# dbolya/yolact

Measured on AMD Instinct MI355X. Metric: images/sec (550x550, batch 8 per GPU), YOLACT yolact_resnet50 forward + Detect (Fast NMS), higher is better.
Workload: dtype f32 (fp32 in / fp32 accumulate / fp32 out; 93 % of the GEMM time on fp16x2 tiles = every fp32 operand as two fp16 pieces by round to nearest (22 significant bits + 2 signs: exact for ~2/3 of all fp32 values, one fp32 ulp otherwise), 3 exact piece products per product on the fp16 matrix pipe; measure

## Files before the change

yolact_amd/csrc/wgemm.hip:

```cpp
#include "common.h"
#include <stdlib.h>
#include <type_traits>
#include "../../include/yolact_amd.h"

int ymi_internal_prof_begin(double flops, int tile, int kind, hipStream_t s);
void ymi_internal_prof_end(int idx, hipStream_t s);

namespace {

typedef __attribute__((address_space(3))) void *lds_ptr_t;
typedef _Float16 f16x8 __attribute__((ext_vector_type(8)));
typedef unsigned u32x4 __attribute__((ext_vector_type(4)));
constexpr unsigned OOB = 0x80000000u;

constexpr int BM = 128, BN = 256;
constexpr int A_BYTES = 2 * BM * 64, B_BYTES = 2 * BN * 64, STAGE = A_BYTES + B_BYTES, NST = 3;
constexpr int OFF_SC = NST * STAGE, WG_LDS = OFF_SC + 2 * BN * 4;
constexpr int NPC = 12;

struct WgParams {
  const char *v, *u;
  const float *uinv, *x_amax;
  float *m;
  long v_gs, u_gs, m_gs;
  unsigned v_plane, u_plane;
  int G, T, C, Ng, cout_pad, tiles_m, tiles_n, nitems;
  float amax_mul;
  unsigned long long *trace;
  int abl;
};

__global__ __launch_bounds__(512, 2) void wgemm_k(const WgParams p) {
#if defined(__HIP_DEVICE_COMPILE__)
  __shared__ __attribute__((aligned(16))) char lds[WG_LDS];
  const int t = threadIdx.x, lane = t & 63, wave = __builtin_amdgcn_readfirstlane(t >> 6);
  const bool producer = wave >= 4;
  const int lr = lane & 31, hh = lane >> 5;
  const int nk = p.C >> 5;
  const int nb = (int)gridDim.x, b0 = (int)blockIdx.x;
  const int my_items = (p.nitems - b0 + nb - 1) / nb;
  const int nsteps = my_items * nk;
#ifdef YMI_DIAGNOSTICS
  unsigned long long tr_[8] = {0, 0, 0, 0, 0, 0, 0, 0};
  const bool tracing = p.trace != nullptr;
  tr_[0] = __builtin_amdgcn_s_memtime();
#endif
#define WG_WAIT_VM(N) asm volatile("s_waitcnt vmcnt(%0)" ::"n"(N) : "memory")
#define WG_BARRIER() asm volatile("s_waitcnt lgkmcnt(0)\n\ts_barrier" ::: "memory")
  auto decode = [&](int it, int &g, int &tm, int &tn) {
    tn = it % p.tiles_n;
    const int r = it / p.tiles_n;
    tm = r % p.tiles_m;
    g = r / p.tiles_m;
  };

  if (producer) {
    const int pw = wave - 4;
    int a_row[4], a_dst[4], b_row[8], b_dst[8];
    unsigned a_ko[4], b_ko[8];
#pragma unroll
    for (int i = 0; i < 4; ++i) {
      const int q = pw + 4 * i, plane = q >> 3, rg = q & 7;
      const int row = rg * 16 + (lane >> 2), lsl = (lane & 3) ^ ((row >> 2) & 3);
      a_row[i] = row; a_ko[i] = (unsigned)plane * p.v_plane + 16u * lsl; a_dst[i] = plane * (BM * 64) + rg * 1024;
    }
#pragma unroll
    for (int i = 0; i < 8; ++i) {
      const int q = pw + 4 * i, plane = q >> 4, rg = q & 15;
      const int row = rg * 16 + (lane >> 2), lsl = (lane & 3) ^ ((row >> 2) & 3);
      b_row[i] = row; b_ko[i] = (unsigned)plane * p.u_plane + 16u * lsl; b_dst[i] = A_BYTES + plane * (BN * 64) + rg * 1024;
    }
    int ridx = 0, rkc = 0;
    __amdgpu_buffer_rsrc_t vrs, urs, srs;
    unsigned a_vo[4], b_vo[8];
    int sc_par = 0;
    auto open_item = [&](int idx) {
      const bool live = idx < my_items;
      int g = 0, tm = 0, tn = 0;
      decode(live ? b0 + idx * nb : 0, g, tm, tn);
      vrs = __builtin_amdgcn_make_buffer_rsrc((void *)(p.v + (size_t)g * p.v_gs), 0, live ? (int)p.v_gs : 0, 0x00020000);
      urs = __builtin_amdgcn_make_buffer_rsrc((void *)(p.u + (size_t)g * p.u_gs), 0, live ? (int)p.u_gs : 0, 0x00020000);
      srs = __builtin_amdgcn_make_buffer_rsrc((void *)(p.uinv + (size_t)g * p.cout_pad), 0, live ? p.cout_pad * 4 : 0, 0x00020000);
#pragma unroll
      for (int i = 0; i < 4; ++i) {
        const int row = tm * BM + a_row[i];
        a_vo[i] = (live && row < p.T && !(p.abl & 2)) ? a_ko[i] + (unsigned)(row * p.C) * 2u : OOB;
      }
#pragma unroll
      for (int i = 0; i < 8; ++i) {
        const int row = tn * BN + b_row[i];
        b_vo[i] = (live && row < p.cout_pad && !(p.abl & 4)) ? b_ko[i] + (unsigned)(row * p.C) * 2u : OOB;
      }
      const int n = tn * BN + 4 * lane;
      __builtin_amdgcn_raw_ptr_buffer_load_lds(srs, (lds_ptr_t)(lds + OFF_SC + sc_par * (BN * 4)), 16, (live && n < p.cout_pad) ? (unsigned)n * 4u : OOB, 0, 0, 0);
      sc_par ^= 1;
    };
    auto request = [&](int stage) {
      if (rkc == 0) open_item(ridx);
      char *dst = lds + stage * STAGE;
      const unsigned so = (unsigned)rkc * 64u;
#pragma unroll
      for (int i = 0; i < 4; ++i) __builtin_amdgcn_raw_ptr_buffer_load_lds(vrs, (lds_ptr_t)(dst + a_dst[i]), 16, a_vo[i], so, 0, 0);
#pragma unroll
      for (int i = 0; i < 8; ++i) __builtin_amdgcn_raw_ptr_buffer_load_lds(urs, (lds_ptr_t)(dst + b_dst[i]), 16, b_vo[i], so, 0, 0);
      if (++rkc == nk) { rkc = 0; ++ridx; }
    };
    request(0);
    request(1);
    WG_WAIT_VM(NPC);
#ifdef YMI_DIAGNOSTICS
    tr_[1] = __builtin_amdgcn_s_memtime();
#endif
    WG_BARRIER();
    int st = 2;
    for (int s = 0; s < nsteps; ++s) {
      request(st);
      st = st == 2 ? 0 : st + 1;
#ifdef YMI_DIAGNOSTICS
      const unsigned long long a_ = tracing ? __builtin_amdgcn_s_memtime() : 0ull;
#endif
      WG_WAIT_VM(NPC);
#ifdef YMI_DIAGNOSTICS
      const unsigned long long b_ = tracing ? __builtin_amdgcn_s_memtime() : 0ull;
#endif
      WG_BARRIER();
#ifdef YMI_DIAGNOSTICS
      if (tracing) { tr_[2] += b_ - a_; tr_[3] += __builtin_amdgcn_s_memtime() - b_; }
#endif
    }
    WG_WAIT_VM(0);
  } else {
    const int wc = wave & 1, wp = wave >> 1;
    const int psw = (lr >> 2) & 3;
    float sA, invA;
    ymi_h2_scale(ymi_amax_read(p.x_amax) * p.amax_mul, sA, invA);
    f32x16 acc[4][2];
#pragma unroll
    for (int i = 0; i < 4; ++i)
#pragma unroll
      for (int j = 0; j < 2; ++j)
#pragma unroll
        for (int r = 0; r < 16; ++r) acc[i][j][r] = 0.f;
    const int uo0 = A_BYTES + (32 * (4 * wc) + lr) * 64 + 16 * ((0 + hh) ^ psw), uo1 = A_BYTES + (32 * (4 * wc) + lr) * 64 + 16 * ((2 + hh) ^ psw);
    const int vo0 = (32 * (2 * wp) + lr) * 64 + 16 * ((0 + hh) ^ psw), vo1 = (32 * (2 * wp) + lr) * 64 + 16 * ((2 + hh) ^ psw);
#ifdef YMI_DIAGNOSTICS
    tr_[1] = __builtin_amdgcn_s_memtime();
#endif
    WG_BARRIER();
    __builtin_amdgcn_s_setprio(1);
    int st = 0, kc = 0, idx = 0, sc_par = 0;
    for (int s = 0; s < nsteps; ++s) {
      const char *sb = lds + st * STAGE;
#pragma unroll
      for (int s2 = 0; s2 < 2; ++s2) {
        const char *ub = sb + (s2 ? uo1 : uo0), *vb = sb + (s2 ? vo1 : vo0);
        f16x8 vh[2], vl[2];
#pragma unroll
        for (int j = 0; j < 2; ++j) {
          vh[j] = *reinterpret_cast<const f16x8 *>(vb + j * 2048);
          vl[j] = *reinterpret_cast<const f16x8 *>(vb + BM * 64 + j * 2048);
        }
#pragma unroll
        for (int ip = 0; ip < 2; ++ip) {
          f16x8 uh[2], ul[2];
#pragma unroll
          for (int ii = 0; ii < 2; ++ii) {
            uh[ii] = *reinterpret_cast<const f16x8 *>(ub + (2 * ip + ii) * 2048);
            ul[ii] = *reinterpret_cast<const f16x8 *>(ub + BN * 64 + (2 * ip + ii) * 2048);
          }
#pragma unroll
          for (int pr = 0; pr < 3; ++pr)
#pragma unroll
            for (int ii = 0; ii < 2; ++ii)
#pragma unroll
              for (int j = 0; j < 2; ++j)
#ifdef YMI_DIAGNOSTICS
                if (!(p.abl & 8))
#endif
                acc[2 * ip + ii][j] = __builtin_amdgcn_mfma_f32_32x32x16_f16(pr == 0 ? ul[ii] : uh[ii], pr == 1 ? vl[j] : vh[j], acc[2 * ip + ii][j], 0, 0, 0);
        }
      }
      st = st == 2 ? 0 : st + 1;
      if (++kc == nk) {
        kc = 0;
        int g, tm, tn;
        decode(b0 + idx * nb, g, tm, tn);
        ++idx;
        const float *sc = reinterpret_cast<const float *>(lds + OFF_SC + sc_par * (BN * 4));
        sc_par ^= 1;
        float *mg = p.m + (size_t)g * p.m_gs;
#pragma unroll
        for (int j = 0; j < 2; ++j) {
          const int row = tm * BM + 32 * (2 * wp + j) + lr;
          const bool rok = row < p.T;
#pragma unroll
          for (int i = 0; i < 4; ++i)
#pragma unroll
            for (int gq = 0; gq < 4; ++gq) {
              const int nl = 32 * (4 * wc + i) + 8 * gq + 4 * hh, n = tn * BN + nl;
              const f32x4 s4 = *reinterpret_cast<const f32x4 *>(sc + nl);
              f32x4 v;
#pragma unroll
              for (int e = 0; e < 4; ++e) { v[e] = acc[i][j][4 * gq + e] * (s4[e] * invA); acc[i][j][4 * gq + e] = 0.f; }
#ifdef YMI_DIAGNOSTICS
              if (p.abl & 1) continue;
              if (p.abl & 16) { if (rok && n < p.Ng) __builtin_nontemporal_store(v, reinterpret_cast<f32x4 *>(mg + (size_t)row * p.Ng + n)); continue; }
#endif
              if (rok && n < p.Ng) *reinterpret_cast<f32x4 *>(mg + (size_t)row * p.Ng + n) = v;
            }
        }
      }
#ifdef YMI_DIAGNOSTICS
      const unsigned long long a_ = tracing ? __builtin_amdgcn_s_memtime() : 0ull;
#endif
      WG_BARRIER();
#ifdef YMI_DIAGNOSTICS
      if (tracing) tr_[3] += __builtin_amdgcn_s_memtime() - a_;
#endif
    }
    __builtin_amdgcn_s_setprio(0);
  }
#undef WG_WAIT_VM
#undef WG_BARRIER
#ifdef YMI_DIAGNOSTICS
  if (tracing) {
    asm volatile("s_waitcnt vmcnt(0)" ::: "memory");
    tr_[5] = __builtin_amdgcn_s_memtime();
    if (lane == 0 && (wave == 0 || wave == 4)) {
      unsigned long long *o_ = p.trace + 32 * (size_t)blockIdx.x + (wave == 0 ? 0 : 16);
#pragma unroll
      for (int i = 0; i < 8; ++i) o_[i] = tr_[i];
      o_[14] = (unsigned long long)nsteps;
      o_[15] = 1;
    }
  }
#endif
#endif
}

}

int ymi_internal_wgemm(const void *v, const void *u, const float *uinv, const float *x_amax, float amax_mul, float *m, int G, long T,
                       int C, int Ng, int cout_pad, double prof_flops, int prof_kind, hipStream_t s) {
  if (!v || !u || !uinv || !x_amax || !m) return YMI_ENULL;
  if (C % 32 != 0 || C < 64 || (Ng & 3) || G <= 0 || T <= 0) return YMI_ESHAPE;
  if (T * (long)C * 4 >= (1L << 31) || (long)cout_pad * C * 4 >= (1L << 31) || T * (long)Ng >= (1L << 29)) return YMI_ESHAPE;
  if ((((uintptr_t)v) | ((uintptr_t)u) | ((uintptr_t)m) | ((uintptr_t)uinv)) & 15) return YMI_ESHAPE;
  WgParams p;
  p.v = (const char *)v; p.u = (const char *)u; p.uinv = uinv; p.x_amax = x_amax; p.m = m;
  p.v_plane = (unsigned)(T * C * 2); p.v_gs = 2L * T * C * 2;
  p.u_plane = (unsigned)((long)cout_pad * C * 2); p.u_gs = 2L * cout_pad * C * 2;
  p.m_gs = T * (long)Ng;
  p.G = G; p.T = (int)T; p.C = C; p.Ng = Ng; p.cout_pad = cout_pad;
  p.tiles_m = (int)((T + BM - 1) / BM); p.tiles_n = (Ng + BN - 1) / BN; p.nitems = G * p.tiles_m * p.tiles_n;
  p.amax_mul = amax_mul;
  p.trace = nullptr; p.abl = 0;
#ifdef YMI_DIAGNOSTICS
  { const char *e = getenv("YMI_WGEMM_ABLATE"); p.abl = e ? atoi(e) : 0; }
  { const char *e = getenv("YMI_WGEMM_TRACE"); p.trace = e ? (unsigned long long *)strtoull(e, nullptr, 0) : nullptr; }
#endif
  int dev = 0, cus = 256;
  hipGetDevice(&dev);
  hipDeviceGetAttribute(&cus, hipDeviceAttributeMultiprocessorCount, dev);
  const int pr = ymi_internal_prof_begin(prof_flops, YMI_TILE_H2 | YMI_TILE_WG_128x256, prof_kind, s);
  hipLaunchKernelGGL(wgemm_k, dim3((unsigned)(p.nitems < cus ? p.nitems : cus)), dim3(512), 0, s, p);
  const int rc = ymi_launch_status();
  ymi_internal_prof_end(pr, s);
  return rc;
}
```

Before: 2307.

## Add weight-stationary wgemm variant keeping U tile in registers for small C

Adds a second GEMM kernel for C of 64, 128 or 256. Each block holds its 256-column slice of the weight operand (U) in registers for the whole K range and streams a contiguous range of M tiles, so weights are loaded once per block instead of once per output tile. The host picks this path when its per-block tile count is not much worse than the round-robin scheduler's, and an environment variable can force the old path. The cost is heavy register use for the resident U fragments (lower occupancy, 256 threads with no producer waves) and possible load imbalance when M tiles split unevenly across blocks.

After: 2349 (median of 6 runs). +1.8%, better.

```diff
diff --git a/yolact_amd/csrc/wgemm.hip b/yolact_amd/csrc/wgemm.hip
--- a/yolact_amd/csrc/wgemm.hip
+++ b/yolact_amd/csrc/wgemm.hip
@@ -1,4 +1,5 @@
 #include "common.h"
+#include <stdio.h>
 #include <stdlib.h>
 #include <type_traits>
 #include "../../include/yolact_amd.h"
@@ -25,6 +26,7 @@
   long v_gs, u_gs, m_gs;
   unsigned v_plane, u_plane;
   int G, T, C, Ng, cout_pad, tiles_m, tiles_n, nitems;
+  int bpc;
   float amax_mul;
   unsigned long long *trace;
   int abl;
@@ -232,6 +234,205 @@
       for (int i = 0; i < 8; ++i) o_[i] = tr_[i];
       o_[14] = (unsigned long long)nsteps;
       o_[15] = 1;
+    }
+  }
+#endif
+#endif
+}
+
+constexpr int US_NST = 3, US_OFF_SC = US_NST * A_BYTES, US_OFF_U = US_OFF_SC + BN * 4, US_LDS = US_OFF_U + US_NST * B_BYTES;
+constexpr int US_NPC = 4;
+
+template <int NK, bool NOMFMA = false>
+__global__ __launch_bounds__(256) void wgemm_us_k(const WgParams p) {
+#if defined(__HIP_DEVICE_COMPILE__)
+  __shared__ __attribute__((aligned(16))) char lds[US_LDS];
+  const int t = threadIdx.x, lane = t & 63, wave = __builtin_amdgcn_readfirstlane(t >> 6);
+  const int lr = lane & 31, hh = lane >> 5;
+  const int lb = ymi_xcd_remap((int)blockIdx.x, (int)gridDim.x);
+  const int gc = lb / p.bpc, jb = lb % p.bpc;
+  const int g = gc / p.tiles_n, tn = gc % p.tiles_n;
+  const int tm0 = jb * p.tiles_m / p.bpc, tm1 = (jb + 1) * p.tiles_m / p.bpc;
+#ifdef YMI_DIAGNOSTICS
+  unsigned long long tr_[8] = {0, 0, 0, 0, 0, 0, 0, 0};
+  const bool tracing = p.trace != nullptr;
+  tr_[0] = __builtin_amdgcn_s_memtime();
+#endif
+#define WG_WAIT_VM(N) asm volatile("s_waitcnt vmcnt(%0)" ::"n"(N) : "memory")
+#define WG_BARRIER() asm volatile("s_waitcnt lgkmcnt(0)\n\ts_barrier" ::: "memory")
+  int a_row[4], a_dst[4];
+  unsigned a_ko[4], a_vo[4], a_vn[4];
+#pragma unroll
+  for (int i = 0; i < 4; ++i) {
+    const int q = wave + 4 * i, plane = q >> 3, rg = q & 7;
+    const int row = rg * 16 + (lane >> 2), lsl = (lane & 3) ^ ((row >> 2) & 3);
+    a_row[i] = row; a_ko[i] = (unsigned)plane * p.v_plane + 16u * lsl; a_dst[i] = plane * (BM * 64) + rg * 1024;
+  }
+  const __amdgpu_buffer_rsrc_t vrs = __builtin_amdgcn_make_buffer_rsrc((void *)(p.v + (size_t)g * p.v_gs), 0, (int)p.v_gs, 0x00020000);
+  auto tile_offsets = [&](int tm, unsigned (&vo)[4]) {
+#pragma unroll
+    for (int i = 0; i < 4; ++i) {
+      const int row = tm * BM + a_row[i];
+      vo[i] = (tm < tm1 && row < p.T && !(p.abl & 2)) ? a_ko[i] + (unsigned)(row * p.C) * 2u : OOB;
+    }
+  };
+  auto piece = [&](int stage, const unsigned (&vo)[4], int kc, int i) {
+    __builtin_amdgcn_raw_ptr_buffer_load_lds(vrs, (lds_ptr_t)(lds + stage * A_BYTES + a_dst[i]), 16, vo[i], (unsigned)kc * 64u, 0, 0);
+  };
+  auto request = [&](int stage, const unsigned (&vo)[4], int kc) {
+#pragma unroll
+    for (int i = 0; i < 4; ++i) piece(stage, vo, kc, i);
+  };
+  if (t < 64) {
+    const int n = tn * BN + 4 * t;
+    f32x4 s4 = {0.f, 0.f, 0.f, 0.f};
+    if (n < p.cout_pad) s4 = *reinterpret_cast<const f32x4 *>(p.uinv + (size_t)g * p.cout_pad + n);
+    *reinterpret_cast<f32x4 *>(lds + US_OFF_SC + 16 * t) = s4;
+  }
+  f16x8 u[2][2][2 * NK];
+  const __amdgpu_buffer_rsrc_t urs = __builtin_amdgcn_make_buffer_rsrc((void *)(p.u + (size_t)g * p.u_gs), 0, (int)p.u_gs, 0x00020000);
+  int b_dst[8];
+  unsigned b_vo[8];
+#pragma unroll
+  for (int i = 0; i < 8; ++i) {
+    const int q = wave + 4 * i, plane = q >> 4, rg = q & 15;
+    const int row = rg * 16 + (lane >> 2), lsl = (lane & 3) ^ ((row >> 2) & 3), grow = tn * BN + row;
+    b_dst[i] = plane * (BN * 64) + rg * 1024;
+    b_vo[i] = (grow < p.cout_pad && !(p.abl & 4)) ? (unsigned)plane * p.u_plane + 16u * lsl + (unsigned)(grow * p.C) * 2u : OOB;
+  }
+  auto upiece = [&](int stage, int kc, int i) {
+    __builtin_amdgcn_raw_ptr_buffer_load_lds(urs, (lds_ptr_t)(lds + US_OFF_U + stage * B_BYTES + b_dst[i]), 16, b_vo[i], (unsigned)kc * 64u, 0, 0);
+  };
+  tile_offsets(tm0, a_vo);
+#pragma unroll
+  for (int c = 0; c < 2; ++c) {
+    request(c, a_vo, c);
+#pragma unroll
+    for (int i = 0; i < 8; ++i) upiece(c, c, i);
+  }
+  float sA, invA;
+  ymi_h2_scale(ymi_amax_read(p.x_amax) * p.amax_mul, sA, invA);
+  f32x16 acc[2][4];
+#pragma unroll
+  for (int i = 0; i < 2; ++i)
+#pragma unroll
+    for (int j = 0; j < 4; ++j)
+#pragma unroll
+      for (int r = 0; r < 16; ++r) acc[i][j][r] = 0.f;
+  const int psw = (lr >> 2) & 3;
+  const int vo0 = lr * 64 + 16 * ((0 + hh) ^ psw), vo1 = lr * 64 + 16 * ((2 + hh) ^ psw);
+  const float *sc = reinterpret_cast<const float *>(lds + US_OFF_SC);
+  float *mg = p.m + (size_t)g * p.m_gs;
+  WG_WAIT_VM(0);
+#ifdef YMI_DIAGNOSTICS
+  tr_[1] = __builtin_amdgcn_s_memtime();
+#endif
+  WG_BARRIER();
+  __builtin_amdgcn_s_setprio(1);
+  f16x8 fa[4], fb[4];
+  auto rd = [&](f16x8 (&f)[4], int stage, int s2, int jp) {
+    const char *vb = lds + stage * A_BYTES + (s2 ? vo1 : vo0) + jp * 4096;
+    f[0] = *reinterpret_cast<const f16x8 *>(vb);
+    f[1] = *reinterpret_cast<const f16x8 *>(vb + 2048);
+    f[2] = *reinterpret_cast<const f16x8 *>(vb + BM * 64);
+    f[3] = *reinterpret_cast<const f16x8 *>(vb + BM * 64 + 2048);
+  };
+  auto mm = [&](const f16x8 (&f)[4], int ks, int jp) {
+    if constexpr (NOMFMA) {
+      asm volatile("" ::"v"(f[0]), "v"(f[1]), "v"(f[2]), "v"(f[3]));
+      return;
+    }
+#pragma unroll
+    for (int pr = 0; pr < 3; ++pr)
+#pragma unroll
+      for (int i = 0; i < 2; ++i)
+#pragma unroll
+        for (int jj = 0; jj < 2; ++jj)
+          acc[i][2 * jp + jj] = __builtin_amdgcn_mfma_f32_32x32x16_f16(u[i][pr == 0 ? 1 : 0][ks], f[pr == 1 ? 2 + jj : jj], acc[i][2 * jp + jj], 0, 0, 0);
+  };
+#define WG_PIN() __builtin_amdgcn_sched_barrier(0)
+  int st = 0;
+  rd(fa, 0, 0, 0);
+  auto tile = [&](auto first_, int tm) {
+    constexpr bool FIRST = decltype(first_)::value;
+    tile_offsets(tm + 1, a_vn);
+#pragma unroll
+    for (int kc = 0; kc < NK; ++kc) {
+      const int rs = st == 0 ? 2 : st - 1, rk = kc + 2 < NK ? kc + 2 : kc + 2 - NK;
+      const unsigned (&rv)[4] = kc + 2 < NK ? a_vo : a_vn;
+      const bool ureq = FIRST && kc + 2 < NK;
+      if constexpr (FIRST) {
+        const char *ub = lds + US_OFF_U + (kc % 3) * B_BYTES + (64 * wave + lr) * 64;
+#pragma unroll
+        for (int i = 0; i < 2; ++i)
+#pragma unroll
+          for (int pl = 0; pl < 2; ++pl)
+#pragma unroll
+            for (int s2 = 0; s2 < 2; ++s2)
+              u[i][pl][2 * kc + s2] = *reinterpret_cast<const f16x8 *>(ub + pl * (BN * 64) + i * 2048 + 16 * ((2 * s2 + hh) ^ psw));
+      }
+      rd(fb, st, 0, 1); piece(rs, rv, rk, 0); if (ureq) { upiece((kc + 2) % 3, kc + 2, 0); upiece((kc + 2) % 3, kc + 2, 1); } WG_PIN();
+      mm(fa, 2 * kc, 0); WG_PIN();
+      rd(fa, st, 1, 0); piece(rs, rv, rk, 1); if (ureq) { upiece((kc + 2) % 3, kc + 2, 2); upiece((kc + 2) % 3, kc + 2, 3); } WG_PIN();
+      mm(fb, 2 * kc, 1); WG_PIN();
+      rd(fb, st, 1, 1); piece(rs, rv, rk, 2); if (ureq) { upiece((kc + 2) % 3, kc + 2, 4); upiece((kc + 2) % 3, kc + 2, 5); } WG_PIN();
+      mm(fa, 2 * kc + 1, 0); WG_PIN();
+      piece(rs, rv, rk, 3); if (ureq) { upiece((kc + 2) % 3, kc + 2, 6); upiece((kc + 2) % 3, kc + 2, 7); }
+      st = st == 2 ? 0 : st + 1;
+#ifdef YMI_DIAGNOSTICS
+      const unsigned long long a_ = tracing ? __builtin_amdgcn_s_memtime() : 0ull;
+#endif
+      if (ureq) WG_WAIT_VM(US_NPC + 8); else WG_WAIT_VM(US_NPC);
+#ifdef YMI_DIAGNOSTICS
+      const unsigned long long b_ = tracing ? __builtin_amdgcn_s_memtime() : 0ull;
+#endif
+      WG_BARRIER();
+#ifdef YMI_DIAGNOSTICS
+      if (tracing) { tr_[2] += b_ - a_; tr_[3] += __builtin_amdgcn_s_memtime() - b_; }
+#endif
+      rd(fa, st, 0, 0); WG_PIN();
+      mm(fb, 2 * kc + 1, 1); WG_PIN();
+    }
+#pragma unroll
+    for (int j = 0; j < 4; ++j) {
+      const int row = tm * BM + 32 * j + lr;
+      const bool rok = row < p.T;
+#pragma unroll
+      for (int i = 0; i < 2; ++i)
+#pragma unroll
+        for (int gq = 0; gq < 4; ++gq) {
+          const int nl = 64 * wave + 32 * i + 8 * gq + 4 * hh, n = tn * BN + nl;
+          const f32x4 s4 = *reinterpret_cast<const f32x4 *>(sc + nl);
+          f32x4 v;
+#pragma unroll
+          for (int e = 0; e < 4; ++e) { v[e] = acc[i][j][4 * gq + e] * (s4[e] * invA); acc[i][j][4 * gq + e] = 0.f; }
+#ifdef YMI_DIAGNOSTICS
+          if (p.abl & 1) continue;
+          if (p.abl & 16) { if (rok && n < p.Ng) __builtin_nontemporal_store(v, reinterpret_cast<f32x4 *>(mg + (size_t)row * p.Ng + n)); continue; }
+#endif
+          if (rok && n < p.Ng) *reinterpret_cast<f32x4 *>(mg + (size_t)row * p.Ng + n) = v;
+        }
+    }
+#pragma unroll
+    for (int i = 0; i < 4; ++i) a_vo[i] = a_vn[i];
+  };
+  tile(std::true_type{}, tm0);
+  for (int tm = tm0 + 1; tm < tm1; ++tm) tile(std::false_type{}, tm);
+  __builtin_amdgcn_s_setprio(0);
+  WG_WAIT_VM(0);
+#undef WG_WAIT_VM
+#undef WG_BARRIER
+#undef WG_PIN
+#ifdef YMI_DIAGNOSTICS
+  if (tracing) {
+    tr_[5] = __builtin_amdgcn_s_memtime();
+    if (lane == 0 && wave == 0) {
+      unsigned long long *o_ = p.trace + 32 * (size_t)blockIdx.x;
+#pragma unroll
+      for (int i = 0; i < 8; ++i) { o_[i] = tr_[i]; o_[16 + i] = tr_[i]; }
+      o_[13] = o_[29] = 1;
+      o_[14] = o_[30] = (unsigned long long)((tm1 - tm0) * NK);
+      o_[15] = o_[31] = 1;
     }
   }
 #endif
@@ -262,8 +463,29 @@
   int dev = 0, cus = 256;
   hipGetDevice(&dev);
   hipDeviceGetAttribute(&cus, hipDeviceAttributeMultiprocessorCount, dev);
+  const int gcs = G * p.tiles_n;
+  p.bpc = cus / gcs < 1 ? 1 : (cus / gcs < p.tiles_m ? cus / gcs : p.tiles_m);
+  const int run_us = (p.tiles_m + p.bpc - 1) / p.bpc, run_rr = (p.nitems + cus - 1) / cus;
+  const char *force = getenv("YMI_WGEMM_STREAM_U");
+  const bool us = (C == 256 || C == 128 || C == 64) && 4 * run_us <= 5 * run_rr && !(force && atoi(force) != 0);
+  if (getenv("YMI_WGEMM_LOG"))
+    fprintf(stderr, "wgemm: %s G=%d T=%ld C=%d Ng=%d blocks=%d\n", us ? "u-stationary" : "u-streamed", G, T, C, Ng,
+            us ? gcs * p.bpc : (p.nitems < cus ? p.nitems : cus));
   const int pr = ymi_internal_prof_begin(prof_flops, YMI_TILE_H2 | YMI_TILE_WG_128x256, prof_kind, s);
-  hipLaunchKernelGGL(wgemm_k, dim3((unsigned)(p.nitems < cus ? p.nitems : cus)), dim3(512), 0, s, p);
+  if (us) {
+    const dim3 grid((unsigned)(gcs * p.bpc));
+#ifdef YMI_DIAGNOSTICS
+    if (p.abl & 8) {
+      if (C == 256) hipLaunchKernelGGL((wgemm_us_k<8, true>), grid, dim3(256), 0, s, p);
+      else if (C == 128) hipLaunchKernelGGL((wgemm_us_k<4, true>), grid, dim3(256), 0, s, p);
+      else hipLaunchKernelGGL((wgemm_us_k<2, true>), grid, dim3(256), 0, s, p);
+    } else
+#endif
+    if (C == 256) hipLaunchKernelGGL(wgemm_us_k<8>, grid, dim3(256), 0, s, p);
+    else if (C == 128) hipLaunchKernelGGL(wgemm_us_k<4>, grid, dim3(256), 0, s, p);
+    else hipLaunchKernelGGL(wgemm_us_k<2>, grid, dim3(256), 0, s, p);
+  } else
+    hipLaunchKernelGGL(wgemm_k, dim3((unsigned)(p.nitems < cus ? p.nitems : cus)), dim3(512), 0, s, p);
   const int rc = ymi_launch_status();
   ymi_internal_prof_end(pr, s);
   return rc;
```
